# musevlt/muse-psfr

Measured on AMD Instinct MI355X. Metric: PSFs/sec (row x lambda) on 512^2 grid, 35 lambda, higher is better.
Workload: dtype f64 PSD->structure function, per-lambda OTF f32 -> split-fp16 MFMA (fp32 accumulate), f64 fit

## Files before the change

muse_psfr_amd/csrc/kernels.h:

```cpp
#pragma once
#include <hip/hip_runtime.h>
#include <stdint.h>

namespace mpsfr {

constexpr int NS = 40;
constexpr int NSH = NS / 2 + 1;
constexpr int KS = 41;
constexpr int NAO = 80;
constexpr int kNH = NAO / 2 + 1;
constexpr int NFIT = 16;
constexpr int NFIT_ELL = 24;
constexpr int NFIT_PSF = 16;
constexpr int NFIT_GROUP = 48;
constexpr int METRIC_MAX = 16;
constexpr int METRIC_HEAD = 8;
constexpr int KHAT = 33 * 64;
constexpr int MAXLGS = 4;

struct TaskPar {
    double r0m53;
    double inv_l0sq;
    double cn2_0;
    double cn2_1;
// ... 110 lines not shown
size_t mf_dminb_bytes(int N, int ntask);
int mf_block_count(int N);
void launch_mf_tables(hipStream_t s, int N, int nl, const LamPar* d_lp, const void* d_tw64,
                      void* d_E, void* d_G);
void launch_mf_tel(hipStream_t s, int N, const void* d_tel, float* d_tl2, float* d_tlb);
void launch_peak_floor(hipStream_t s, int N, int ntask, int ndir, const void* d_D0t, const float* d_tl2, float c2min,
                       float tier_half, float floor_nominal, float* d_thrf);
void launch_otf_mfma(hipStream_t s, int N, int ntask, int ndir, int nl, const void* d_D0t,
                     const float* d_tl2, const LamPar* d_lp, const void* d_E, const void* d_G,
                     const int* d_vkeep, const float* d_dminb, const float* d_tlb, float thr,
                     void* d_pre, const int* d_order = nullptr, void* d_clk = nullptr, const float* d_thrf = nullptr);
size_t mf2_own_bytes(int N, int ntask, int nl);
size_t mf2_uni_bytes(int N, int ntask, int nl);
size_t mf2_sched_bytes(int N, int ntask, int nl, int permax);
size_t mf2_part_bytes(int N, int ntask, int nl);
void mf2_groups(int nl, int permax, int* per, int* ngr);
void launch_mf_prep(hipStream_t s, int N, int ntask, int nl, int permax, const LamPar* d_lp,
                    const float* d_dminb, const float* d_tlb, float thr, float thr_floor, float thr_mid,
                    float tier_half, const void* d_D0t, const float* d_tl2, void* d_own,
                    void* d_uni, void* d_sched, const float* d_dlin = nullptr);
void launch_otf_mfma2(hipStream_t s, int N, int ntask, int nl, int permax, int ncu, const void* d_D0t,
                      const float* d_tl2, const LamPar* d_lp, const void* d_E, const void* d_G,
                      const void* d_own, const void* d_uni, void* d_sched, void* d_part, void* d_pre,
                      void* d_clk = nullptr, hipEvent_t ev_start = nullptr, hipEvent_t ev_stop = nullptr);
void launch_gtable(hipStream_t s, int N, int nl, const LamPar* d_lp, const void* d_tw64,
                   int* d_samp_p, void* d_samp_a, void* d_G, bool f64);
void launch_moffat_kernels(hipStream_t s, int nker, const double* d_gamma, const double* d_alpha,
                           void* d_out, bool f64);
void launch_otf_rowfft(hipStream_t s, int N, int ntask, int ndir, int nl, const void* d_D0t,
                       const void* d_tel, const LamPar* d_lp, const int* d_samp_p,
                       const void* d_samp_a, const void* d_xtab, void* d_Tq, const void* d_tw64,
                       bool f64, bool fast_exp, const int* d_vkeep);
bool otf_uses_r16(int N, bool f64, int nl, int ndir);
size_t xtab_bytes(int nl);
void launch_xtab(hipStream_t s, int N, int nl, const int* d_samp_p, const void* d_samp_a,
                 const void* d_tw64, void* d_xtab);
void launch_colpass(hipStream_t s, int N, int ntask, int nl, const void* d_Tq, const void* d_G,
                    void* d_pre, bool f64, const int* d_vkeep);
void launch_conv(hipStream_t s, int ntask, int nl, const void* d_pre, const void* d_ktt,
                 const void* d_kmuse, double* d_fin, bool f64, int tdiv = 1);
void launch_khat(hipStream_t s, int nker, const double* d_gamma, const double* d_alpha,
                 void* d_khat, bool f64 = false);
void launch_conv_fft(hipStream_t s, int ntask, int nl, const void* d_pre, const void* d_khat_tt,
                     const void* d_khat_muse, void* d_fin, bool fin_f32, bool f64 = false, int tdiv = 1);
void launch_fit(hipStream_t s, int nstamp, const void* d_stamps, bool stamps_f32, double* d_fit,
                bool f64, int sum_ntask = 0, int sum_nl = 0, double* d_sum = nullptr, int sum_accumulate = 0);
void launch_stamp_sum(hipStream_t s, int ntask, int nl, const void* d_fin, bool fin_f32, double* d_sum,
                      int accumulate);
void launch_fit_ell(hipStream_t s, int nstamp, const double* d_stamps, double* d_fit, bool f64);
void launch_fit_obs(hipStream_t s, int nstamp, const double* d_stamps, const double* d_var, int flags, double* d_fit,
                    bool f64);
void launch_fit_psf(hipStream_t s, int nstamp, const double* d_stamps, const double* d_var, int npsf,
                    const double* d_psf, const int32_t* d_index, const double* d_shift, int flags, double* d_fit,
                    bool f64);
void launch_fit_group(hipStream_t s, int nstamp, int nsrc, const double* d_stamps, const double* d_var, int npsf,
                      const double* d_psf, const int32_t* d_index, const double* d_shift, int flags, double* d_fit,
                      bool f64);
void launch_fit_spec(hipStream_t s, int nstar, int nl, const double* d_cubes, const double* d_var, int npsf,
                     const double* d_psf, const int32_t* d_index, const double* d_shift, const double* d_x, int flags,
                     double* d_fit, bool f64);
void launch_stamp_metrics(hipStream_t s, int nstamp, const double* d_stamps, const double* d_centers, int nrad,
                          const double* radii, int nbox, const double* boxes, int nfrac, const double* fractions,
                          double* d_out);
void launch_cut_stamps(hipStream_t s, int ny, int nx, const double* d_image, const double* d_var, int nstar,
                       const int32_t* d_origin, double* d_stamps, double* d_var_out);
struct StarList {
    int nstar, npsf;
// ... 59 lines not shown
```

muse_psfr_amd/csrc/mf_common.h:

```cpp
#pragma once
#include "device_common.h"

namespace mpsfr {
namespace {

typedef _Float16 h8 __attribute__((ext_vector_type(8)));
typedef _Float16 h4 __attribute__((ext_vector_type(4)));
typedef _Float16 h2 __attribute__((ext_vector_type(2)));
typedef float f4 __attribute__((ext_vector_type(4)));
typedef float f2 __attribute__((ext_vector_type(2)));

constexpr int MTL = 16;
constexpr int KBL = 32;
constexpr int NCT = 3;
constexpr int NJT = 2;
constexpr float kShift = 15.0f;
constexpr int kTabShift = 9;

__host__ __device__ constexpr int mf_nks(int N) { return N / KBL; }
__host__ __device__ constexpr int mf_nmt(int N) { return (N / 2 + 1 + MTL - 1) / MTL; }

[[maybe_unused]] __device__ __forceinline__ void split16(float x, _Float16* hi, _Float16* lo) {
    const _Float16 h = (_Float16)x;
    *hi = h;
    *lo = (_Float16)(x - (float)h);
}

[[maybe_unused]] __device__ __forceinline__ f4 mm16(f4 c, h4 ahi, h4 alo, h4 bhi, h4 blo) {
    c = __builtin_amdgcn_mfma_f32_16x16x16f16(alo, bhi, c, 0, 0, 0);
    c = __builtin_amdgcn_mfma_f32_16x16x16f16(ahi, blo, c, 0, 0, 0);
    return __builtin_amdgcn_mfma_f32_16x16x16f16(ahi, bhi, c, 0, 0, 0);
}

[[maybe_unused]] __device__ __forceinline__ void write_stamp(const f4* P0, const f4* Q0, const f4* R2x,
                                                            const f4* R2y, int lr, int lk,
                                                            float* __restrict__ out) {
    float va[2 * NJT * 4], vb[2 * NJT * 4];
    float part = 0.f;
#pragma unroll
    for (int jt = 0; jt < NJT; ++jt) {
        const int jj = 16 * jt + lr;
        const bool jok = jj < NSH;
        const float mj = (jj >= 1 && jj <= NS / 2 - 1) ? 1.f : 0.f;
#pragma unroll
        for (int r = 0; r < 4; ++r) {
            const float qhi = __shfl_xor(R2y[jt][r], 32, 64);
#pragma unroll
            for (int top = 0; top < 2; ++top) {
                const int row = 4 * lk + r;
                const int ii = top ? 16 + row : row;
                const bool ok = jok && (top ? row < 5 : true);
                const float Pv = top ? R2x[jt][r] : P0[jt][r];
                const float Qv = top ? qhi : Q0[jt][r];
                const float pa = ok ? fmaxf(Pv + Qv, 0.f) : 0.f;
                const float pb = ok ? fmaxf(Pv - Qv, 0.f) : 0.f;
                const float mi = (ii >= 1 && ii <= NS / 2 - 1) ? 1.f : 0.f;
                part += pa * (1.f + mi * mj) + pb * (mi + mj);
                va[(top * NJT + jt) * 4 + r] = pa;
                vb[(top * NJT + jt) * 4 + r] = pb;
            }
        }
    }
    const double tot = wave_sum((double)part);
    const float inv = (float)(1.0 / tot);
#pragma unroll
    for (int top = 0; top < 2; ++top)
#pragma unroll
        for (int jt = 0; jt < NJT; ++jt)
#pragma unroll
            for (int r = 0; r < 4; ++r) {
                const int row = 4 * lk + r, ii = top ? 16 + row : row, jj = 16 * jt + lr;
                if (jj >= NSH || (top && row >= 5)) continue;
                const float pa = va[(top * NJT + jt) * 4 + r] * inv, pb = vb[(top * NJT + jt) * 4 + r] * inv;
                const bool mi = ii >= 1 && ii <= NS / 2 - 1, mj = jj >= 1 && jj <= NS / 2 - 1;
                out[ii * NS + jj] = pa;
                if (mi) out[(NS - ii) * NS + jj] = pb;
                if (mj) out[ii * NS + NS - jj] = pb;
                if (mi && mj) out[(NS - ii) * NS + NS - jj] = pa;
            }
}

[[maybe_unused]] __device__ __forceinline__ bool part_col(int jt, int lr) { return 16 * jt + lr < NSH; }
[[maybe_unused]] __device__ __forceinline__ bool part_r2x(int lk) { return lk < 2; }
[[maybe_unused]] __device__ __forceinline__ bool part_r2y(int lk) { return lk >= 2; }

constexpr int kT2 = 8;

#ifndef MPSFR_MF_BASE_NOP
#define MPSFR_MF_BASE_NOP 4
#endif
#ifndef MF_XSTR
#define MF_STR(x_) #x_
#define MF_XSTR(x_) MF_STR(x_)
#endif

[[maybe_unused]] __device__ __forceinline__ void glds16s(const void* sbase, unsigned voff, unsigned lds_dst) {
    unsigned keep;
    asm volatile(
        "s_nop " MF_XSTR(MPSFR_MF_BASE_NOP) "\n\ts_mov_b32 %0, m0\n\ts_mov_b32 m0, %3\n\ts_nop 0\n\tglobal_load_lds_dwordx4 %1, %2\n\ts_mov_b32 m0, %0"
        : "=&s"(keep)
        : "v"(voff), "s"(sbase), "s"(lds_dst)
        : "memory");
// ... 27 lines not shown
```

muse_psfr_amd/csrc/mpsfr_api.cpp:

```cpp
#include "../../include/mpsfr.h"

#include <hip/hip_runtime.h>

#include <algorithm>
#include <chrono>
#include <cmath>
#include <cstdarg>
#include <cstdio>
#include <cstring>
#include <string>
#include <thread>
#include <vector>

#include "coeff_l0_table.h"
#include "kernels.h"

using namespace mpsfr;

namespace {

thread_local std::string g_err;

constexpr float kMfFloorLog2 = -29.01f;

// ... 17 lines not shown

const char* kKernelNames[K_COUNT] = {
    "ao_tables", "tel_otf", "psd_rowfft", "colfft_dphi", "gtable",
    "moffat_kernels", "otf_rowfft", "colpass", "conv", "fit", "stamp_sum", "vkeep", "otf_mfma", "mf_prep",
    "patch", "dphi_series"};

struct DevBuf {
    void* p = nullptr;
    size_t cap = 0;
};

struct Pending {
    int id;
    hipEvent_t a, b;
};

}

struct mpsfr_ctx {
    int device = 0, N = 0, dimpsf = 0, prec = 0, ncu = 256;
    int reserve_mf = -1, reserve_a = -1;
    bool head_fusion = true;
    bool support_skip = true;
    double pixscale = 0.2;
    bool f64 = false;
    hipStream_t stream = nullptr;
    int chunk_tasks = 0;
    bool fast_exp = true;
    bool profile = false;
    int prof_only = -1;
    int prof_every = 1;
    unsigned prof_count[64] = {};
    bool fft_conv = true;
    int prune_fixed = 0;
    double prune_eps = 1.0e-9;
    double prune_eps_f64 = 1.0e-13;
    bool otf_mfma = true;
    bool mf_floor = true;
    int mf_kernel = 2;
    int mf_permax = 6;
    double mf_mid_log2 = -18.01;
    double mf_floor_log2 = kMfFloorLog2;
    double tier_eps = 4.0e-6;
    bool mf_clock = false;
    int stage_a = 1;
    DevBuf mfclk;
// ... 84 lines not shown
        std::vector<double> sums;
        std::vector<long> tickets;
        double* user_sum = nullptr;
    } multi;
    long ticket_next = 0;
    long d0t_clears = 0;
    double host_seconds = 0.0;
    long host_calls = 0;
    std::vector<double> cache_lbda;
    int cache_lbda_mode = -1;
    const void* cache_G_ptr = nullptr;
    const void* cache_kmuse_ptr = nullptr;
    const void* cache_xtab_ptr = nullptr;
    bool cache_xtab_valid = false;
    const void* cache_etab_ptr = nullptr;
    const void* cache_gtab_ptr = nullptr;
    bool cache_mf_valid = false;
    std::vector<unsigned char> cache_geom;
    const void* cache_ao_ptr = nullptr;
    int last_ndir = 0, last_nl = 0, last_chunk_tasks = 0, last_lane = 0;
    int last_ntab = 2;
    int last_gpp = 1;
    bool last_mf = false, last_pruned = false, last_mf2 = false, last_dlin = false;
    float last_thr_blk = 0.f;
    bool last_floor_per_task = false;
    std::vector<double> last_lpc;
    float last_thr[7] = {0.f, 0.f, 0.f, 0.f, 0.f, 0.f, 0.f};
    double prof_ms[K_COUNT] = {0};
    long prof_n[K_COUNT] = {0};
    std::vector<Pending> pending;
    std::vector<hipEvent_t> pool;
};

namespace {

size_t rsize(const mpsfr_ctx* c) { return c->f64 ? sizeof(double) : sizeof(float); }

int ensure(mpsfr_ctx* c, DevBuf& b, size_t bytes) {
    if (bytes <= b.cap) return MPSFR_OK;
    if (b.p) {
        HIPCHK(hipDeviceSynchronize());
        HIPCHK(hipFree(b.p));
        b.p = nullptr;
        b.cap = 0;
    }
    const size_t want = bytes + bytes / 8;
// ... 495 lines not shown
    } else if (!strcmp(key, "prune_eps")) {
        if (!(value >= 0.0) || value > 1.0e-3) return fail(MPSFR_E_INVALID, "prune_eps must be in [0, 1e-3]");
        c->prune_eps = value;
    } else if (!strcmp(key, "otf_mfma")) {
        c->otf_mfma = value != 0.0;
    } else if (!strcmp(key, "mf_floor")) {
        c->mf_floor = value != 0.0;
    } else if (!strcmp(key, "mf_kernel")) {
        if (value != 1.0 && value != 2.0) return fail(MPSFR_E_INVALID, "mf_kernel must be 1 or 2");
        c->mf_kernel = (int)value;
    } else if (!strcmp(key, "cold_stagger")) {
        c->cold_stagger = (int)value;
    } else if (!strcmp(key, "mf_permax")) {
        if (value != (int)value || value < 1.0 || value > 7.0) return fail(MPSFR_E_INVALID, "mf_permax must be 1..7");
        c->mf_permax = (int)value;
    } else if (!strcmp(key, "persist_reserve") || !strcmp(key, "persist_reserve_mf") || !strcmp(key, "persist_reserve_a")) {
        if (value != (int)value || value < -1.0 || value > 128.0) return fail(MPSFR_E_INVALID, "%s must be -1 (automatic) or 0..128", key);
        if (key[15] == '\0' || key[16] == 'm') c->reserve_mf = (int)value;
        if (key[15] == '\0' || key[16] == 'a') c->reserve_a = (int)value;
    } else if (!strcmp(key, "support_skip")) {
        c->support_skip = value != 0.0;
    } else if (!strcmp(key, "head_fusion")) {
        c->head_fusion = value != 0.0;
    } else if (!strcmp(key, "param_copy")) {
        c->param_copy_kernel = value != 0.0;
    } else if (!strcmp(key, "tier_eps")) {
        if (!(value >= 0.0)) return fail(MPSFR_E_INVALID, "tier_eps must be >= 0 (inf: tiers without a budget)");
        c->tier_eps = value;
    } else if (!strcmp(key, "mf_floor_log2")) {
        c->mf_floor_log2 = value;
    } else if (!strcmp(key, "mf_mid_log2")) {
        c->mf_mid_log2 = value;
    } else if (!strcmp(key, "stage_a")) {
        if (value != 0.0 && value != 1.0 && value != 2.0)
            return fail(MPSFR_E_INVALID, "stage_a must be 0 (full-size transforms), 1 (automatic) or 2 (series + patch)");
        c->stage_a = (int)value;
    } else if (!strcmp(key, "mf_clock")) {
        c->mf_clock = value != 0.0;
        if (c->mf_clock) {
            const int rc = ensure(c, c->mfclk, (size_t)65536 * 8 * 8 * sizeof(unsigned long long));
            if (rc) return rc;
            HIPCHK(hipMemset(c->mfclk.p, 0, c->mfclk.cap));
        }
    } else if (!strcmp(key, "pipeline_calls")) {
        c->pipeline_calls = value != 0.0;
    } else if (!strcmp(key, "fft_conv")) {
// ... 1033 lines not shown
        }
        if (!c->lsum_done) HIPCHK(hipEventCreateWithFlags(&c->lsum_done, hipEventDisableTiming));
        HIPCHK(hipEventRecord(c->lsum_done, s));
        c->lsum_busy = true;
    }
    if (!m.lean) {
        HIPCHK(hipEventRecord(sl.call_done, s));
        if (!c->stream_tail) HIPCHK(hipEventCreateWithFlags(&c->stream_tail, hipEventDisableTiming));
    }
    sl.call_pending = true;
    sl.last_lane = m.lean ? L.index(0) : -1;
    sl.has_event = !m.zero;
    return MPSFR_OK;
}

static void remember_call(mpsfr_ctx* c, const CallPrep& p, bool dlin) {
    c->last_ndir = p.ndir;
    c->last_gpp = p.gpp;
    c->last_nl = p.nl;
    c->last_mf = p.mf;
    c->last_mf2 = p.mf2;
    c->last_pruned = p.th.prune;
    c->last_dlin = dlin;
    c->last_thr_blk = p.th.thr_blk;
    c->last_floor_per_task = p.th.floor_per_task;
    const float thr[7] = {p.th.thr_eps, p.th.thr_floor, p.th.thr_mid, p.th.tier_half, p.th.thr_blk, p.th.thr_sum,
                          p.th.c2min};
    for (int k = 0; k < 7; ++k) c->last_thr[k] = thr[k];
    c->last_lpc.resize(p.nl);
    for (int l = 0; l < p.nl; ++l) c->last_lpc[l] = p.lp[l].c;
}


struct Chunk {
    int t0, tc;
    int j;
    bool accumulate;
    bool shared;
};

static int d0t_begin(mpsfr_ctx* c, mpsfr_ctx::Lane& ln, bool skip_form, int leaves) {
    if (ln.d0t_stale == 2 || (ln.d0t_stale == 1 && skip_form)) {
        HIPCHK(hipMemsetAsync(ln.D0t.p, 0, ln.D0t.cap, ln.stream));
        ln.d0t_stale = 0;
        ++c->d0t_clears;
    }
// ... 22 lines not shown
            }
            launch_patch(ls, N, ntd, ndir, d.tp + t0, (const double*)c->aotab.p, cfit, c->stwk.p,
                         (double*)ln.pP.p, ln.pT.p, (double*)ln.psp.p, c->f64, kh, d.mix(t0));
        }
        ProfScope ps(c, K_DPHI_SERIES, ls);
        launch_dphi_series(ls, N, ntd, ndir, d.tp + t0, ln.pT.p, (const double*)ln.psp.p, c->scoef.p,
                           c->stwk.p, scale2, ln.D0t.p, p.th.prune ? (float*)ln.dlin.p : nullptr, c->f64,
                           msched, persist_grid(c, ln, c->reserve_a, ck.shared),
                           c->support_skip ? (const unsigned*)c->ssup.p : nullptr);
    } else {
        {
            ProfScope ps(c, K_PSD_ROWFFT, ls);
            launch_psd_rowfft(ls, N, ntd, ndir, d.tp + t0, (const double*)c->aotab.p, cfit, ln.C.p,
                              c->tw64.p, (double*)ln.s00.p, c->f64, d.mix(t0));
        }
        ProfScope ps(c, K_COLFFT_DPHI, ls);
        launch_colfft_dphi(ls, N, ntd, ln.C.p, (const double*)ln.s00.p, scale2, ln.D0t.p,
                           c->f64, c->tw64.p, msched);
    }
    return MPSFR_OK;
}

static int stage_b(mpsfr_ctx* c, mpsfr_ctx::Lane& ln, const CallPrep& p, const DevParams& d, const Chunk& ck,
                   bool from_lines, CallLanes& L) {
    hipStream_t ls = ln.stream;
    const int N = p.N, nl = p.nl, ndb = p.ndb, ntd = ck.tc * p.ndir;
    const int tb = ck.tc * p.gpp;
    const Thresholds& th = p.th;
    const bool prune = th.prune;
    if (p.mf2) {
        ProfScope ps(c, K_MF_PREP, ls);
        const bool lines = prune && from_lines;
        if (prune && !lines) launch_dmin(ls, N, ntd, ln.D0t.p, (float*)ln.dmin.p, (float*)ln.dblk.p);
        launch_mf_prep(ls, N, tb, nl, c->mf_permax, d.lp, (prune && !lines) ? (const float*)ln.dblk.p : nullptr,
                       (const float*)c->tlb.p, th.thr_eps, th.thr_floor, th.thr_mid, th.tier_half, ln.D0t.p,
                       (const float*)c->tl2.p, ln.mown.p, ln.muni.p, ln.msched.p,
                       lines ? (const float*)ln.dlin.p : nullptr);
    } else if (prune) {
        ProfScope ps(c, p.mf ? K_MF_PREP : K_VKEEP, ls);
        if (from_lines) launch_dmin16(ls, N, ntd, (const float*)ln.dlin.p, (float*)ln.dmin.p, (float*)ln.dblk.p);
        else launch_dmin(ls, N, ntd, ln.D0t.p, (float*)ln.dmin.p, (float*)ln.dblk.p, c->f64);
        launch_vkeep(ls, N, tb, ndb, nl, d.lp, (const float*)ln.dmin.p, (const float*)ln.dblk.p,
                     (const float*)c->tlmax.p, th.thr_sum, (int*)ln.vkeep.p, c->prune_fixed,
                     p.mf ? (float*)ln.dminb.p : nullptr);
        if (p.mf) launch_task_order(ls, tb, nl, (const int*)ln.vkeep.p, (int*)ln.order.p);
    }
    const int* d_vkeep = prune ? (const int*)ln.vkeep.p : nullptr;
    if (int rc = stagger_here(c, L, 2, ln)) return rc;
    if (p.mf2) {
        ProfScope ps(c, K_OTF_MFMA, ls, false);
        launch_otf_mfma2(ls, N, tb, nl, c->mf_permax, persist_grid(c, ln, c->reserve_mf, ck.shared), ln.D0t.p,
                         (const float*)c->tl2.p, d.lp, c->etab.p, c->gtab.p, ln.mown.p, ln.muni.p, ln.msched.p,
                         ln.mpart.p, ln.pre.p, c->mf_clock ? c->mfclk.p : nullptr, ps.a, ps.b);
    } else if (p.mf) {
        ProfScope ps(c, K_OTF_MFMA, ls);
        if (th.floor_per_task)
            launch_peak_floor(ls, N, tb, ndb, ln.D0t.p, (const float*)c->tl2.p, th.c2min, th.tier_half, th.thr_floor,
                              (float*)ln.thrf.p);
        launch_otf_mfma(ls, N, tb, ndb, nl, ln.D0t.p, (const float*)c->tl2.p, d.lp, c->etab.p,
                        c->gtab.p, d_vkeep, prune ? (const float*)ln.dminb.p : nullptr,
                        (const float*)c->tlb.p, th.thr_blk, ln.pre.p,
                        prune ? (const int*)ln.order.p : nullptr, c->mf_clock ? c->mfclk.p : nullptr,
                        th.floor_per_task ? (const float*)ln.thrf.p : nullptr);
    } else {
        {
            ProfScope ps(c, K_OTF_ROWFFT, ls);
            launch_otf_rowfft(ls, N, tb, ndb, nl, ln.D0t.p, c->tel.p, d.lp,
                              (const int*)c->samp_p.p, c->samp_a.p, c->xtab.p, ln.Tq.p, c->tw64.p,
                              c->f64, c->fast_exp, d_vkeep);
        }
        ProfScope ps(c, K_COLPASS, ls);
        launch_colpass(ls, N, tb, nl, ln.Tq.p, c->G.p, ln.pre.p, c->f64, d_vkeep);
    }
    return MPSFR_OK;
}

static int chunk_tail(mpsfr_ctx* c, mpsfr_ctx::Lane& ln, const CallPrep& p, const DevParams& d, const CallOuts& o,
                      const Chunk& ck, int NL) {
    hipStream_t ls = ln.stream;
    const int nl = p.nl, nsum = p.nsum, t0 = ck.t0, tc = ck.tc;
    const int tb = tc * p.gpp;
    const size_t per_stamp = kStampPix;
    const bool fin_f32 = p.band ? (p.fft_conv && !c->f64)
                                : (p.fft_conv && !c->f64 && !o.d_fin_all && !(o.psf && !o.dev));
    void* d_fin = o.d_fin_all ? (void*)(o.d_fin_all + (size_t)t0 * nsum * per_stamp) : ln.fin.p;
    {
        ProfScope ps(c, K_CONV, ls);
        const char* ktt = d.ktt + (size_t)t0 * p.ksz;
        if (p.fft_conv) launch_conv_fft(ls, tb, nl, ln.pre.p, ktt, c->kmuse.p, d_fin, fin_f32, c->f64, p.gpp);
        else launch_conv(ls, tb, nl, ln.pre.p, ktt, c->kmuse.p, (double*)d_fin, c->f64, p.gpp);
    }
    void* d_res = d_fin;
    bool res_f32 = fin_f32;
    if (p.band) {
        ProfScope ps(c, K_STAMP_SUM, ls);
        double* d_band = (o.dev && o.psf) ? o.psf + (size_t)t0 * nsum * per_stamp : (double*)ln.band.p;
        launch_band_reduce(ls, tb, nl, p.nout, d_fin, fin_f32, d.bw, d_band);
        d_res = d_band;
        res_f32 = false;
    }
    double* lsum = !o.sum ? nullptr : NL > 1 ? (double*)c->lsum.p + (size_t)ck.j * nsum * per_stamp : o.d_sum;
    if (o.fit) {
        ProfScope ps(c, K_FIT, ls);
        launch_fit(ls, tb * p.nout, d_res, res_f32, o.d_fit_all + (size_t)t0 * nsum * NFIT, c->f64,
                   o.sum ? tc : 0, nsum, o.sum ? lsum : nullptr, ck.accumulate ? 1 : 0);
    } else if (o.sum) {
        ProfScope ps(c, K_STAMP_SUM, ls);
        launch_stamp_sum(ls, tc, nsum, d_res, res_f32, lsum, ck.accumulate ? 1 : 0);
    }
    HIPCHK(hipGetLastError());
    if (!o.dev && o.psf) {
        HIPCHK(hipMemcpyAsync(o.psf + (size_t)t0 * nsum * per_stamp, d_res,
                              (size_t)tc * nsum * per_stamp * sizeof(double), hipMemcpyDeviceToHost, ls));
// ... 31 lines not shown
    mpsfr_ctx::Ticket* tk = nullptr;
    if (a.on_device == 2 && (rc = ticket_begin(c, p, o, tk))) return rc;
    const bool pipelined = c->pipeline_calls && o.dev;
    CallLanes L;
    if ((rc = lanes_begin(c, p.ntask, pipeline_chunk_tasks(c, p, !pipelined), pipelined, L))) return rc;
    const Markers marks(c, o.dev, tk != nullptr, L.NL);
    hipStream_t s0 = L.at(c, 0).stream;
    std::vector<unsigned char> ao_key = ao_cache_key(p.g, p.ly, a.mask_rec, a.mask_res);
    bool ao_cached = false, lam_cached = false;
    if ((rc = size_ao_tables(c, p, ao_key, ao_cached))) return rc;
    const Blob blob(p, a.mask_rec && !ao_cached);
    mpsfr_ctx::Slot* sl = nullptr;
    if ((rc = slot_acquire(c, blob.bytes, (size_t)p.ntask * p.ksz, sl, clock.blocked))) return rc;
    blob.fill(sl->host, p, a.mask_rec, a.mask_res);
    const void* outs[3] = {o.dev ? (const void*)o.psf : nullptr, o.dev ? (const void*)o.sum : nullptr,
                           o.dev ? (const void*)o.fit : nullptr};
    if ((rc = queue_call_waits(c, L, *sl, outs))) return rc;
    const std::vector<double> lb_key(a.lbda_nm, a.lbda_nm + a.nl);
    if ((rc = size_wavelength_tables(c, p, lb_key, lam_cached))) return rc;
    if ((rc = send_params(c, *sl, s0, blob.bytes, marks))) return rc;
    const DevParams d = blob.views(*sl, p);
    if ((rc = refresh_tables(c, s0, p, d, ao_cached ? nullptr : &ao_key, lam_cached ? nullptr : &lb_key))) return rc;
    const bool fuse_khat = c->head_fusion && p.series && p.fft_conv;
    launch_tiptilt(c, s0, p, d, *sl, fuse_khat);
    for (int j = 0; j < L.NL; ++j)
        if ((rc = size_lane(c, L.at(c, j), p, L.TC, STAGE_A | STAGE_B | STAGE_TAIL, p.band && !(o.dev && o.psf))))
            return rc;
    if ((rc = size_outputs(c, p, L.NL, o))) return rc;
    if ((rc = share_tables(c, L))) return rc;
    rc = for_each_chunk(c, p.ntask, L, lanes_are_shared(c, L), [&](mpsfr_ctx::Lane& ln, const Chunk& ck) {
        int r;
        if ((r = stage_a(c, ln, p, d, ck, fuse_khat))) return r;
        if ((r = stagger_here(c, L, 1, ln))) return r;
        if ((r = stage_b(c, ln, p, d, ck, p.th.prune && p.series, L))) return r;
        return chunk_tail(c, ln, p, d, o, ck, L.NL);
    });
    if (rc) return rc;
    if ((rc = call_end(c, L, *sl, marks, outs, p.nsum, o.sum ? o.d_sum : nullptr))) return rc;
    remember_call(c, p, p.th.prune && p.series);
    if (tk && (rc = ticket_finish(c, tk))) return rc;
    if (!o.dev) {
        hipStream_t s = c->stream;
        if (o.fit)
            HIPCHK(hipMemcpyAsync(o.fit, o.d_fit_all, (size_t)p.ntask * p.nsum * NFIT * sizeof(double),
                                  hipMemcpyDeviceToHost, s));
        if (o.sum)
            HIPCHK(hipMemcpyAsync(o.sum, o.d_sum, (size_t)p.nsum * kStampPix * sizeof(double), hipMemcpyDeviceToHost, s));
        HIPCHK(hipStreamSynchronize(s));
    }
    clock.finish(c);
    return MPSFR_OK;
}

struct ScopedBuf : DevBuf {
    ~ScopedBuf() { release(*this); }
};

enum : unsigned { TABLES_AO = 1, TABLES_WAVELENGTH = 2 };
static const void* const kNoOuts[3] = {nullptr, nullptr, nullptr};

struct StageCall {
    CallLanes L;
// ... 1040 lines not shown
    if (!strcmp(what, "ao_tables")) {
        n = (size_t)2 * c->last_ndir * (c->last_ntab + 1) * NAO * NAO;
        src = c->aotab.p;
    } else if (!strcmp(what, "tel")) {
        n = (size_t)H1 * N;
        src = c->tel.p;
        is_real_r = true;
    } else if (!strcmp(what, "dphi0")) {
        n = (size_t)c->last_chunk_tasks * c->last_ndir * H1 * N;
        src = c->lane[c->last_lane].D0t.p;
        is_real_r = true;
    } else if (!strcmp(what, "dlin")) {
        if (!c->last_dlin)
            return fail(MPSFR_E_INVALID, "no line minima in the last call (prune_eps = 0, or stage A did not run in "
                                         "its series form)");
        n = (size_t)c->last_chunk_tasks * c->last_ndir * H1 * (N / 32);
        if (n > capacity) return fail(MPSFR_E_INVALID, "capacity %zu < %zu", capacity, n);
        std::vector<float> tmp(n);
        HIPCHK(hipMemcpy(tmp.data(), c->lane[c->last_lane].dlin.p, n * sizeof(float), hipMemcpyDeviceToHost));
        for (size_t i = 0; i < n; ++i) out[i] = (double)tmp[i];
        return (long)n;
    } else if (!strcmp(what, "pre")) {
        n = (size_t)c->last_chunk_tasks * c->last_gpp * c->last_nl * NS * NS;
        src = c->lane[c->last_lane].pre.p;
        is_real_r = true;
    } else if (!strcmp(what, "mf_work")) {
        if (capacity < 3) return fail(MPSFR_E_INVALID, "capacity %zu < 3", capacity);
        if (!c->last_mf) return fail(MPSFR_E_INVALID, "the last call did not use the matrix-core kernel");
        const int tc = c->last_chunk_tasks * c->last_gpp, nl = c->last_nl, npair = (nl + 1) / 2;
        const int nks = N / 32, nmt = (H1 + 15) / 16, nb = nmt * nks;
        const mpsfr_ctx::Lane& ln = c->lane[c->last_lane];
        std::vector<int> vk((size_t)tc * npair);
        std::vector<float> dm((size_t)tc * nb), tb((size_t)nb);
        if (c->last_pruned && !c->last_mf2) {
            HIPCHK(hipMemcpy(vk.data(), ln.vkeep.p, vk.size() * sizeof(int), hipMemcpyDeviceToHost));
            HIPCHK(hipMemcpy(dm.data(), ln.dminb.p, dm.size() * sizeof(float), hipMemcpyDeviceToHost));
            HIPCHK(hipMemcpy(tb.data(), c->tlb.p, tb.size() * sizeof(float), hipMemcpyDeviceToHost));
        }
        double steps = 0.0, tiles = 0.0, steps_full = 0.0, steps_mid = 0.0, steps_union = -1.0, steps_support = -1.0;
        if (c->last_mf2) {
            std::vector<unsigned long long> own((size_t)tc * nl * nmt * 2);
            HIPCHK(hipMemcpy(own.data(), ln.mown.p, own.size() * sizeof(unsigned long long), hipMemcpyDeviceToHost));
            for (size_t i = 0; i < own.size(); i += 2) {
                const int nf = __builtin_popcountll(own[i]), nm = __builtin_popcountll(own[i + 1]);
                steps_full += nf;
                steps_mid += nm;
                tiles += (nf + nm) > 0;
// ... 236 lines not shown
```

muse_psfr_amd/csrc/otf_mfma2.hip:

```cpp
#include <hip/hip_ext.h>
#include "mf_common.h"

namespace mpsfr {

namespace {

typedef unsigned long long u64;

constexpr int kTW = 4;
constexpr int kStage2 = kT2 * 4096;
constexpr int kSlab = 6 * 1024;

struct MaskArgs {
    int N, nl, per, ngr;
    const LamPar* lp;
    const float* dminb;
    const float* dlin;
    const float* tlb;
    float thr, thr_mid;
    float thr_floor, tier_half;
    const float* D0t;
    const float* tl2;
    u64* own;
    u64* uni;
// ... 616 lines not shown
                    const float* d_dminb, const float* d_tlb, float thr, float thr_floor, float thr_mid,
                    float tier_half, const void* d_D0t, const float* d_tl2, void* d_own,
                    void* d_uni, void* d_sched, const float* d_dlin) {
    MaskArgs a;
    a.dlin = d_dlin;
    a.thr_floor = thr_floor; a.tier_half = tier_half;
    a.D0t = (const float*)d_D0t; a.tl2 = d_tl2;
    a.N = N; a.nl = nl;
    mf2_groups(nl, permax, &a.per, &a.ngr);
    a.lp = d_lp; a.dminb = d_dminb; a.tlb = d_tlb;
    a.thr = thr; a.thr_mid = thr_mid;
    a.own = (u64*)d_own; a.uni = (u64*)d_uni;
    a.ksum = a.uni + (size_t)ntask * nl * mf_nmt(N);
    a.kuni = a.ksum + (size_t)ntask * nl * mf2_nsw(N);
    const SchedPtrs p = sched_ptrs(d_sched, ntask, nl);
    a.gsw = p.gsw; a.sched = p.sched; a.items = p.items;
    a.cap = (int)mf2_cap(N, ntask, a.ngr);
    hipLaunchKernelGGL(k_mf_prep, dim3(a.ngr, ntask), dim3(64 * a.per), 0, s, a);
}

void launch_otf_mfma2(hipStream_t s, int N, int ntask, int nl, int permax, int ncu, const void* d_D0t,
                      const float* d_tl2, const LamPar* d_lp, const void* d_E, const void* d_G,
                      const void* d_own, const void* d_uni, void* d_sched, void* d_part, void* d_pre,
                      void* d_clk, hipEvent_t ev_start, hipEvent_t ev_stop) {
    Mf2Args a;
    a.N = N; a.ntask = ntask; a.nl = nl;
    mf2_groups(nl, permax, &a.per, &a.ngr);
    a.D0t = (const float*)d_D0t; a.tl2 = d_tl2; a.lp = d_lp;
    a.E = (const h8*)d_E; a.G = (const h4*)d_G;
    a.own = (const u64*)d_own; a.uni = (const u64*)d_uni;
    a.ksum = a.uni + (size_t)ntask * nl * mf_nmt(N);
    a.kuni = a.ksum + (size_t)ntask * nl * mf2_nsw(N);
    const SchedPtrs p = sched_ptrs(d_sched, ntask, nl);
    a.sched = p.sched; a.items = p.items;
    a.cap = (int)mf2_cap(N, ntask, a.ngr);
    a.part = (f4*)d_part;
    a.clk = (unsigned long long*)d_clk;
    int lg = 0;
    while ((1 << lg) < N) ++lg;
    a.tq_scale = 1.0f / ((float)(1 << lg) * (float)(1 << kTabShift));
    a.pre = (float*)d_pre;
    const int maxitems = ntask * a.ngr * (int)mf2_nsw(N);
    const int nwg = ncu < maxitems ? ncu : maxitems;
    const size_t sm = 2 * (size_t)kStage2 + 2 * (size_t)a.per * kSlab + 64;
    if (permax > 6) {
        allow_smem(k_otf_mfma2<4>, 2 * (size_t)kStage2 + 2 * (size_t)7 * kSlab + 64);
        if (ev_start != nullptr)
            hipExtLaunchKernelGGL(k_otf_mfma2<4>, dim3(nwg), dim3(128 * a.per), (unsigned)sm, s, ev_start, ev_stop, 0, a);
        else
            hipLaunchKernelGGL(k_otf_mfma2<4>, dim3(nwg), dim3(128 * a.per), sm, s, a);
    } else {
        allow_smem(k_otf_mfma2<3>, 2 * (size_t)kStage2 + 2 * (size_t)6 * kSlab + 64);
        if (ev_start != nullptr)
            hipExtLaunchKernelGGL(k_otf_mfma2<3>, dim3(nwg), dim3(128 * a.per), (unsigned)sm, s, ev_start, ev_stop, 0, a);
        else
            hipLaunchKernelGGL(k_otf_mfma2<3>, dim3(nwg), dim3(128 * a.per), sm, s, a);
    }
    hipLaunchKernelGGL(k_mf_finish, dim3(nl, ntask), dim3(64), 0, s, N, nl, a.per, a.ngr, (const int*)p.gsw,
                       (const f4*)a.part, a.pre);
}

}
```

muse_psfr_amd/csrc/stamps.hip:

```cpp
#include "device_common.h"
#include "conv_frames.h"
#include "fit_common.h"
#include <type_traits>

namespace mpsfr {

namespace {

template <typename R>
__global__ void __launch_bounds__(256)
k_moffat_kernels(const double* __restrict__ gam, const double* __restrict__ alp,
                 R* __restrict__ out) {
    __shared__ double part[4];
    __shared__ double tot;
    const int k = blockIdx.x;
    const double g2 = gam[k] * gam[k], al = alp[k];
    double vals[(KS * KS + 255) / 256];
    double s = 0.0;
#pragma unroll
    for (int m = 0; m < (KS * KS + 255) / 256; ++m) {
        const int e = threadIdx.x + m * 256;
        double v = 0.0;
        if (e < KS * KS) {
            const int dy = e / KS - KS / 2, dx = e % KS - KS / 2;
            const double x1 = 1.0 + (double)(dx * dx + dy * dy) / g2;
// ... 76 lines not shown
            const R* __restrict__ krow = kg + a * KS;
#pragma unroll
            for (int b = 0; b < KS; ++b) {
                const R kv = krow[b];
#pragma unroll
                for (int o = 0; o < SW; ++o) part[o] += kv * sv[o - b + 2 * HK];
            }
#pragma unroll
            for (int o = 0; o < SW; ++o) acc[o] += (double)part[o];
        }
        __syncthreads();
        if (pass == 0 && active) {
#pragma unroll
            for (int o = 0; o < SW; ++o) img[(i + HK) * PW + j0 + HK + o] = (R)acc[o];
        }
    }
    if (active) {
        double* out = fin + ((size_t)task * nl + l) * NS * NS + i * NS + j0;
#pragma unroll
        for (int o = 0; o < SW; ++o) out[o] = acc[o];
    }
}

template <typename R, typename TF>
#ifndef MPSFR_CONV_WAVES
#define MPSFR_CONV_WAVES 4
#endif
__global__ void __launch_bounds__(256) __attribute__((amdgpu_waves_per_eu(sizeof(R) == 4 ? MPSFR_CONV_WAVES : 2)))
k_conv_fft(int nl, int tdiv, const R* __restrict__ pre, const cx<R>* __restrict__ khat_tt,
           const cx<R>* __restrict__ khat_muse, TF* __restrict__ fin) {
    extern __shared__ __align__(16) unsigned char conv_smem[];
    cx<R> (*F)[CFP] = reinterpret_cast<cx<R> (*)[CFP]>(conv_smem);
    cx<R> (*bufs)[CFB] = reinterpret_cast<cx<R> (*)[CFB]>(conv_smem + sizeof(cx<R>) * CF * CFP);
    const int l = blockIdx.x, task = blockIdx.y;
    const int slot = threadIdx.x >> 3, t = threadIdx.x & 7;
    Tw64<R> tw;
    tw.init(t);
    const R* src = pre + ((size_t)task * nl + l) * NS * NS;
    cx<R>* buf = bufs[slot];
    cx<R> x[8];
#pragma unroll
    for (int e = 0; e < 8; ++e) {
        const int c = t + 8 * e;
        const bool in = c < NS && slot < NS / 2;
        x[e] = {in ? src[2 * slot * NS + c] : (R)0, in ? src[(2 * slot + 1) * NS + c] : (R)0};
    }
    for (int pass = 0; pass < 2; ++pass) {
        const cx<R>* __restrict__ kh = pass == 0 ? khat_tt + (size_t)(task / tdiv) * (CFH + 1) * CF
                                                     : khat_muse + (size_t)l * (CFH + 1) * CF;
        cx<R> khv[8], khn[8];
#pragma unroll
        for (int e = 0; e < 8; ++e) {
            khv[e] = kh[slot * CF + t + 8 * e];
            khn[e] = slot == 0 ? kh[CFH * CF + t + 8 * e] : cx<R>{(R)0, (R)0};
        }
        __syncthreads();
        if (slot < NS / 2) cf_rows_forward(x, F, buf, tw, slot, t);
        __syncthreads();
        {
            static_assert(fft_last_nbt<CF>() == 1 && fft_last_radix<CF>() == 8, "v[e] is element t + 8 e");
            cx<R> y[8], xin[8], v[8];
#pragma unroll
            for (int e = 0; e < 8; ++e) {
                const int r = t + 8 * e;
                xin[e] = r < NS ? F[r][slot] : cx<R>{(R)0, (R)0};
            }
            fft_forward_regs_lastreg<R, CF, true>(xin, buf, buf, tw.w, t, v);
            if (slot == 0) {
// ... 651 lines not shown
                           (const double*)d_kmuse, d_fin);
    } else {
        const size_t sm = (size_t)(PH * PW) * sizeof(float);
        hipLaunchKernelGGL(k_conv<float>, grid, dim3(256), sm, s, nl, tdiv, (const float*)d_pre,
                           (const float*)d_ktt,
                           (const float*)d_kmuse, d_fin);
    }
}

void launch_khat(hipStream_t s, int nker, const double* d_gamma, const double* d_alpha,
                 void* d_khat, bool f64) {
    if (nker <= 0) return;
    if (f64) {
        allow_smem(k_khat<double>, conv_smem_bytes<double>(true));
        hipLaunchKernelGGL(k_khat<double>, dim3(nker), dim3(256), conv_smem_bytes<double>(true), s, d_gamma,
                           d_alpha, (cx<double>*)d_khat);
    } else {
        hipLaunchKernelGGL(k_khat<float>, dim3(nker), dim3(256), conv_smem_bytes<float>(true), s, d_gamma,
                           d_alpha, (cx<float>*)d_khat);
    }
}

void launch_conv_fft(hipStream_t s, int ntask, int nl, const void* d_pre, const void* d_khat_tt,
                     const void* d_khat_muse, void* d_fin, bool fin_f32, bool f64, int tdiv) {
    const dim3 grid(nl, ntask);
    if (f64) {
        allow_smem((k_conv_fft<double, double>), conv_smem_bytes<double>(false));
        hipLaunchKernelGGL((k_conv_fft<double, double>), grid, dim3(256), conv_smem_bytes<double>(false), s, nl, tdiv,
                           (const double*)d_pre, (const cx<double>*)d_khat_tt, (const cx<double>*)d_khat_muse,
                           (double*)d_fin);
    } else if (fin_f32) {
        hipLaunchKernelGGL((k_conv_fft<float, float>), grid, dim3(256), conv_smem_bytes<float>(false), s, nl, tdiv,
                           (const float*)d_pre, (const cx<float>*)d_khat_tt, (const cx<float>*)d_khat_muse,
                           (float*)d_fin);
    } else {
        hipLaunchKernelGGL((k_conv_fft<float, double>), grid, dim3(256), conv_smem_bytes<float>(false), s, nl, tdiv,
                           (const float*)d_pre, (const cx<float>*)d_khat_tt, (const cx<float>*)d_khat_muse,
                           (double*)d_fin);
    }
}

void launch_fit(hipStream_t s, int nstamp, const void* d_stamps, bool stamps_f32, double* d_fit,
                bool f64, int sum_ntask, int sum_nl, double* d_sum, int sum_accumulate) {
    if (nstamp <= 0) return;
    SumArgs sa = {0, sum_ntask, sum_nl, sum_accumulate, d_sum};
    if (d_sum != nullptr && sum_ntask > 0) {
        const size_t per = (size_t)sum_nl * NS * NS;
        sa.nwg = (int)((per + 64 * MPSFR_FIT_WG - 1) / (64 * MPSFR_FIT_WG));
    }
    const dim3 grid(sa.nwg + (nstamp + MPSFR_FIT_WG - 1) / MPSFR_FIT_WG), blk(64 * MPSFR_FIT_WG);
#ifndef MPSFR_FIT_F64_LM
#define MPSFR_FIT_F64_LM 0
#endif
    if (f64 && MPSFR_FIT_F64_LM)
        hipLaunchKernelGGL((k_fit<double, double>), grid, blk, 0, s, nstamp,
                           (const double*)d_stamps, d_fit, 0.0, sa);
    else if (stamps_f32)
        hipLaunchKernelGGL((k_fit<float, float>), grid, blk, 0, s, nstamp, (const float*)d_stamps,
                           d_fit, (double)MPSFR_POLISH_TOL, sa);
    else
        hipLaunchKernelGGL((k_fit<float, double>), grid, blk, 0, s, nstamp,
// ... 18 lines not shown
```

Before: 20.53 million.

## Fuse MFMA partial-tile reduction into the FFT convolution kernel

The separate k_mf_finish kernel, which summed per-sweep partial tiles into the pre stamps, is removed from the default path. When mf2 and the FFT convolution are both active in f32 mode and outputs stay on the host, the convolution kernel reads the partial tiles itself, reduces them in shared memory and writes the stamp there before its FFT. This saves one kernel launch and the global round trip through pre. A debug readout of 'pre' now runs the finish lazily, and there is extra shared-memory and register pressure in the convolution kernel.

```diff
diff --git a/muse_psfr_amd/csrc/kernels.h b/muse_psfr_amd/csrc/kernels.h
--- a/muse_psfr_amd/csrc/kernels.h
+++ b/muse_psfr_amd/csrc/kernels.h
@@ -156,7 +156,16 @@
 void launch_otf_mfma2(hipStream_t s, int N, int ntask, int nl, int permax, int ncu, const void* d_D0t,
                       const float* d_tl2, const LamPar* d_lp, const void* d_E, const void* d_G,
                       const void* d_own, const void* d_uni, void* d_sched, void* d_part, void* d_pre,
-                      void* d_clk = nullptr, hipEvent_t ev_start = nullptr, hipEvent_t ev_stop = nullptr);
+                      void* d_clk = nullptr, hipEvent_t ev_start = nullptr, hipEvent_t ev_stop = nullptr,
+                      bool finish = true);
+void launch_mf_finish(hipStream_t s, int N, int ntask, int nl, int permax, const void* d_sched, const void* d_part,
+                      void* d_pre);
+struct MfPartial {
+    const void* part;
+    const int* gsw;
+    int per, ngr, nsw;
+};
+MfPartial mf2_partial(int N, int ntask, int nl, int permax, const void* d_sched, const void* d_part);
 void launch_gtable(hipStream_t s, int N, int nl, const LamPar* d_lp, const void* d_tw64,
                    int* d_samp_p, void* d_samp_a, void* d_G, bool f64);
 void launch_moffat_kernels(hipStream_t s, int nker, const double* d_gamma, const double* d_alpha,
@@ -176,7 +185,8 @@
 void launch_khat(hipStream_t s, int nker, const double* d_gamma, const double* d_alpha,
                  void* d_khat, bool f64 = false);
 void launch_conv_fft(hipStream_t s, int ntask, int nl, const void* d_pre, const void* d_khat_tt,
-                     const void* d_khat_muse, void* d_fin, bool fin_f32, bool f64 = false, int tdiv = 1);
+                     const void* d_khat_muse, void* d_fin, bool fin_f32, bool f64 = false, int tdiv = 1,
+                     const MfPartial* tiles = nullptr);
 void launch_fit(hipStream_t s, int nstamp, const void* d_stamps, bool stamps_f32, double* d_fit,
                 bool f64, int sum_ntask = 0, int sum_nl = 0, double* d_sum = nullptr, int sum_accumulate = 0);
 void launch_stamp_sum(hipStream_t s, int ntask, int nl, const void* d_fin, bool fin_f32, double* d_sum,
diff --git a/muse_psfr_amd/csrc/mf_common.h b/muse_psfr_amd/csrc/mf_common.h
--- a/muse_psfr_amd/csrc/mf_common.h
+++ b/muse_psfr_amd/csrc/mf_common.h
@@ -34,7 +34,7 @@
 
 [[maybe_unused]] __device__ __forceinline__ void write_stamp(const f4* P0, const f4* Q0, const f4* R2x,
                                                             const f4* R2y, int lr, int lk,
-                                                            float* __restrict__ out) {
+                                                            float* __restrict__ out, int share = 0, int nshare = 1) {
     float va[2 * NJT * 4], vb[2 * NJT * 4];
     float part = 0.f;
 #pragma unroll
@@ -66,7 +66,8 @@
 #pragma unroll
     for (int top = 0; top < 2; ++top)
 #pragma unroll
-        for (int jt = 0; jt < NJT; ++jt)
+        for (int jt = 0; jt < NJT; ++jt) {
+            if (nshare > 1 && (top * NJT + jt) % nshare != share) continue;
 #pragma unroll
             for (int r = 0; r < 4; ++r) {
                 const int row = 4 * lk + r, ii = top ? 16 + row : row, jj = 16 * jt + lr;
@@ -78,6 +79,7 @@
                 if (mj) out[ii * NS + NS - jj] = pb;
                 if (mi && mj) out[(NS - ii) * NS + NS - jj] = pa;
             }
+        }
 }
 
 [[maybe_unused]] __device__ __forceinline__ bool part_col(int jt, int lr) { return 16 * jt + lr < NSH; }
diff --git a/muse_psfr_amd/csrc/mpsfr_api.cpp b/muse_psfr_amd/csrc/mpsfr_api.cpp
--- a/muse_psfr_amd/csrc/mpsfr_api.cpp
+++ b/muse_psfr_amd/csrc/mpsfr_api.cpp
@@ -63,6 +63,7 @@
     int reserve_mf = -1, reserve_a = -1;
     bool head_fusion = true;
     bool support_skip = true;
+    int finish_in_conv = -1;
     double pixscale = 0.2;
     bool f64 = false;
     hipStream_t stream = nullptr;
@@ -193,6 +194,7 @@
     int last_ntab = 2;
     int last_gpp = 1;
     bool last_mf = false, last_pruned = false, last_mf2 = false, last_dlin = false;
+    bool last_unfinished = false;
     float last_thr_blk = 0.f;
     bool last_floor_per_task = false;
     std::vector<double> last_lpc;
@@ -734,6 +736,10 @@
         c->support_skip = value != 0.0;
     } else if (!strcmp(key, "head_fusion")) {
         c->head_fusion = value != 0.0;
+    } else if (!strcmp(key, "finish_in_conv")) {
+        if (value != -1.0 && value != 0.0 && value != 1.0)
+            return fail(MPSFR_E_INVALID, "finish_in_conv must be -1 (automatic), 0 or 1");
+        c->finish_in_conv = (int)value;
     } else if (!strcmp(key, "param_copy")) {
         c->param_copy_kernel = value != 0.0;
     } else if (!strcmp(key, "tier_eps")) {
@@ -1813,6 +1819,7 @@
     c->last_mf2 = p.mf2;
     c->last_pruned = p.th.prune;
     c->last_dlin = dlin;
+    c->last_unfinished = false;
     c->last_thr_blk = p.th.thr_blk;
     c->last_floor_per_task = p.th.floor_per_task;
     const float thr[7] = {p.th.thr_eps, p.th.thr_floor, p.th.thr_mid, p.th.tier_half, p.th.thr_blk, p.th.thr_sum,
@@ -1881,7 +1888,7 @@
 }
 
 static int stage_b(mpsfr_ctx* c, mpsfr_ctx::Lane& ln, const CallPrep& p, const DevParams& d, const Chunk& ck,
-                   bool from_lines, CallLanes& L) {
+                   bool from_lines, CallLanes& L, bool finish = true) {
     hipStream_t ls = ln.stream;
     const int N = p.N, nl = p.nl, ndb = p.ndb, ntd = ck.tc * p.ndir;
     const int tb = ck.tc * p.gpp;
@@ -1910,7 +1917,7 @@
         ProfScope ps(c, K_OTF_MFMA, ls, false);
         launch_otf_mfma2(ls, N, tb, nl, c->mf_permax, persist_grid(c, ln, c->reserve_mf, ck.shared), ln.D0t.p,
                          (const float*)c->tl2.p, d.lp, c->etab.p, c->gtab.p, ln.mown.p, ln.muni.p, ln.msched.p,
-                         ln.mpart.p, ln.pre.p, c->mf_clock ? c->mfclk.p : nullptr, ps.a, ps.b);
+                         ln.mpart.p, ln.pre.p, c->mf_clock ? c->mfclk.p : nullptr, ps.a, ps.b, finish);
     } else if (p.mf) {
         ProfScope ps(c, K_OTF_MFMA, ls);
         if (th.floor_per_task)
@@ -1935,7 +1942,7 @@
 }
 
 static int chunk_tail(mpsfr_ctx* c, mpsfr_ctx::Lane& ln, const CallPrep& p, const DevParams& d, const CallOuts& o,
-                      const Chunk& ck, int NL) {
+                      const Chunk& ck, int NL, bool from_tiles = false) {
     hipStream_t ls = ln.stream;
     const int nl = p.nl, nsum = p.nsum, t0 = ck.t0, tc = ck.tc;
     const int tb = tc * p.gpp;
@@ -1946,8 +1953,14 @@
     {
         ProfScope ps(c, K_CONV, ls);
         const char* ktt = d.ktt + (size_t)t0 * p.ksz;
-        if (p.fft_conv) launch_conv_fft(ls, tb, nl, ln.pre.p, ktt, c->kmuse.p, d_fin, fin_f32, c->f64, p.gpp);
-        else launch_conv(ls, tb, nl, ln.pre.p, ktt, c->kmuse.p, (double*)d_fin, c->f64, p.gpp);
+        if (p.fft_conv) {
+            MfPartial tiles = {};
+            if (from_tiles) tiles = mf2_partial(p.N, tb, nl, c->mf_permax, ln.msched.p, ln.mpart.p);
+            launch_conv_fft(ls, tb, nl, ln.pre.p, ktt, c->kmuse.p, d_fin, fin_f32, c->f64, p.gpp,
+                            from_tiles ? &tiles : nullptr);
+        } else {
+            launch_conv(ls, tb, nl, ln.pre.p, ktt, c->kmuse.p, (double*)d_fin, c->f64, p.gpp);
+        }
     }
     void* d_res = d_fin;
     bool res_f32 = fin_f32;
@@ -2025,6 +2038,8 @@
     const DevParams d = blob.views(*sl, p);
     if ((rc = refresh_tables(c, s0, p, d, ao_cached ? nullptr : &ao_key, lam_cached ? nullptr : &lb_key))) return rc;
     const bool fuse_khat = c->head_fusion && p.series && p.fft_conv;
+    const bool tiles_to_conv = p.mf2 && p.fft_conv && !c->f64 &&
+                               (c->finish_in_conv > 0 || (c->finish_in_conv < 0 && !o.dev));
     launch_tiptilt(c, s0, p, d, *sl, fuse_khat);
     for (int j = 0; j < L.NL; ++j)
         if ((rc = size_lane(c, L.at(c, j), p, L.TC, STAGE_A | STAGE_B | STAGE_TAIL, p.band && !(o.dev && o.psf))))
@@ -2035,12 +2050,13 @@
         int r;
         if ((r = stage_a(c, ln, p, d, ck, fuse_khat))) return r;
         if ((r = stagger_here(c, L, 1, ln))) return r;
-        if ((r = stage_b(c, ln, p, d, ck, p.th.prune && p.series, L))) return r;
-        return chunk_tail(c, ln, p, d, o, ck, L.NL);
+        if ((r = stage_b(c, ln, p, d, ck, p.th.prune && p.series, L, !tiles_to_conv))) return r;
+        return chunk_tail(c, ln, p, d, o, ck, L.NL, tiles_to_conv);
     });
     if (rc) return rc;
     if ((rc = call_end(c, L, *sl, marks, outs, p.nsum, o.sum ? o.d_sum : nullptr))) return rc;
     remember_call(c, p, p.th.prune && p.series);
+    c->last_unfinished = tiles_to_conv;
     if (tk && (rc = ticket_finish(c, tk))) return rc;
     if (!o.dev) {
         hipStream_t s = c->stream;
@@ -3127,7 +3143,15 @@
         return (long)n;
     } else if (!strcmp(what, "pre")) {
         n = (size_t)c->last_chunk_tasks * c->last_gpp * c->last_nl * NS * NS;
-        src = c->lane[c->last_lane].pre.p;
+        mpsfr_ctx::Lane& ln = c->lane[c->last_lane];
+        if (c->last_unfinished) {
+            launch_mf_finish(ln.stream, N, c->last_chunk_tasks * c->last_gpp, c->last_nl, c->mf_permax, ln.msched.p,
+                             ln.mpart.p, ln.pre.p);
+            HIPCHK(hipGetLastError());
+            HIPCHK(hipStreamSynchronize(ln.stream));
+            c->last_unfinished = false;
+        }
+        src = ln.pre.p;
         is_real_r = true;
     } else if (!strcmp(what, "mf_work")) {
         if (capacity < 3) return fail(MPSFR_E_INVALID, "capacity %zu < 3", capacity);
diff --git a/muse_psfr_amd/csrc/otf_mfma2.hip b/muse_psfr_amd/csrc/otf_mfma2.hip
--- a/muse_psfr_amd/csrc/otf_mfma2.hip
+++ b/muse_psfr_amd/csrc/otf_mfma2.hip
@@ -662,7 +662,7 @@
 void launch_otf_mfma2(hipStream_t s, int N, int ntask, int nl, int permax, int ncu, const void* d_D0t,
                       const float* d_tl2, const LamPar* d_lp, const void* d_E, const void* d_G,
                       const void* d_own, const void* d_uni, void* d_sched, void* d_part, void* d_pre,
-                      void* d_clk, hipEvent_t ev_start, hipEvent_t ev_stop) {
+                      void* d_clk, hipEvent_t ev_start, hipEvent_t ev_stop, bool finish) {
     Mf2Args a;
     a.N = N; a.ntask = ntask; a.nl = nl;
     mf2_groups(nl, permax, &a.per, &a.ngr);
@@ -696,8 +696,23 @@
         else
             hipLaunchKernelGGL(k_otf_mfma2<3>, dim3(nwg), dim3(128 * a.per), sm, s, a);
     }
-    hipLaunchKernelGGL(k_mf_finish, dim3(nl, ntask), dim3(64), 0, s, N, nl, a.per, a.ngr, (const int*)p.gsw,
-                       (const f4*)a.part, a.pre);
-}
-
-}
+    if (finish) launch_mf_finish(s, N, ntask, nl, permax, d_sched, d_part, d_pre);
+}
+
+MfPartial mf2_partial(int N, int ntask, int nl, int permax, const void* d_sched, const void* d_part) {
+    MfPartial t;
+    t.part = d_part;
+    t.gsw = sched_ptrs(const_cast<void*>(d_sched), ntask, nl).gsw;
+    mf2_groups(nl, permax, &t.per, &t.ngr);
+    t.nsw = (int)mf2_nsw(N);
+    return t;
+}
+
+void launch_mf_finish(hipStream_t s, int N, int ntask, int nl, int permax, const void* d_sched, const void* d_part,
+                      void* d_pre) {
+    const MfPartial t = mf2_partial(N, ntask, nl, permax, d_sched, d_part);
+    hipLaunchKernelGGL(k_mf_finish, dim3(nl, ntask), dim3(64), 0, s, N, nl, t.per, t.ngr, t.gsw, (const f4*)t.part,
+                       (float*)d_pre);
+}
+
+}
diff --git a/muse_psfr_amd/csrc/stamps.hip b/muse_psfr_amd/csrc/stamps.hip
--- a/muse_psfr_amd/csrc/stamps.hip
+++ b/muse_psfr_amd/csrc/stamps.hip
@@ -1,6 +1,7 @@
 #include "device_common.h"
 #include "conv_frames.h"
 #include "fit_common.h"
+#include "mf_common.h"
 #include <type_traits>
 
 namespace mpsfr {
@@ -123,28 +124,107 @@
     }
 }
 
-template <typename R, typename TF>
+struct ConvPart {
+    const f4* part;
+    const int* gsw;
+    int per, ngr, nsw;
+};
+constexpr int kFinTileBytes = 4 * NJT * 64 * (int)sizeof(f4);
+constexpr int kFinBatch = 6;
+static_assert(NJT == 2, "a thread takes the tiles w and 4 + w: both of column tile w & 1");
+static_assert(kFinTileBytes + NS * NS * (int)sizeof(float) <= (int)sizeof(cx<float>) * CF * CFP, "the scratch lives in F");
+
+__device__ __forceinline__ void conv_finish_intake(const ConvPart& cp, int m, int task, int nl, int l,
+                                                   unsigned char* smem) {
+    f4* tiles = reinterpret_cast<f4*>(smem);
+    float* stamp = reinterpret_cast<float*>(smem + kFinTileBytes);
+    const int lane = threadIdx.x & 63, w = threadIdx.x >> 6;
+    const bool col = part_col(w & 1, lane & 15);
+    const bool top = col && (w < 2 ? part_r2x(lane >> 4) : part_r2y(lane >> 4));
+    const f4* pt = cp.part + ((size_t)task * nl + l) * cp.nsw * (4 * NJT * 64);
+    const unsigned e0 = threadIdx.x, e1 = threadIdx.x + 4 * 64;
+    const f4 z = {0.f, 0.f, 0.f, 0.f};
+    int mm = m & ((1 << cp.nsw) - 1);
+    const int n = __builtin_popcount(mm);
+    f4 a[kFinBatch], b[kFinBatch];
+#pragma unroll
+    for (int k = 0; k < kFinBatch; ++k) {
+        const f4* ps = pt + (size_t)(mm != 0 ? __builtin_ctz(mm) : 0) * (4 * NJT * 64);
+        mm &= mm - 1;
+        a[k] = (col && k < n) ? ps[e0] : z;
+        b[k] = (top && k < n) ? ps[e1] : z;
+    }
+    f4 s0 = a[0], s1 = b[0];
+#pragma unroll
+    for (int k = 1; k < kFinBatch; ++k) {
+        const f4 t0 = s0 + a[k], t1 = s1 + b[k];
+        s0 = k < n ? t0 : s0;
+        s1 = k < n ? t1 : s1;
+    }
+#pragma clang loop unroll(disable)
+    while (mm != 0) {
+        const f4* ps = pt + (size_t)__builtin_ctz(mm) * (4 * NJT * 64);
+        mm &= mm - 1;
+        s0 = s0 + (col ? ps[e0] : z);
+        s1 = s1 + (top ? ps[e1] : z);
+    }
+    tiles[threadIdx.x] = s0;
+    tiles[4 * 64 + threadIdx.x] = s1;
+    __syncthreads();
+    {
+        f4 P0[NJT], Q0[NJT], R2x[NJT], R2y[NJT];
+#pragma unroll
+        for (int jt = 0; jt < NJT; ++jt) {
+            P0[jt] = tiles[(0 * NJT + jt) * 64 + lane];
+            Q0[jt] = tiles[(1 * NJT + jt) * 64 + lane];
+            R2x[jt] = tiles[(2 * NJT + jt) * 64 + lane];
+            R2y[jt] = tiles[(3 * NJT + jt) * 64 + lane];
+        }
+        write_stamp(P0, Q0, R2x, R2y, lane & 15, lane >> 4, stamp, w, 4);
+    }
+    __syncthreads();
+}
+
+template <typename R, typename TF, bool FIN = false>
 #ifndef MPSFR_CONV_WAVES
 #define MPSFR_CONV_WAVES 4
 #endif
 __global__ void __launch_bounds__(256) __attribute__((amdgpu_waves_per_eu(sizeof(R) == 4 ? MPSFR_CONV_WAVES : 2)))
 k_conv_fft(int nl, int tdiv, const R* __restrict__ pre, const cx<R>* __restrict__ khat_tt,
-           const cx<R>* __restrict__ khat_muse, TF* __restrict__ fin) {
+           const cx<R>* __restrict__ khat_muse, TF* __restrict__ fin, ConvPart cp) {
+    static_assert(!FIN || sizeof(R) == 4, "partial tiles are a mixed-mode matter");
     extern __shared__ __align__(16) unsigned char conv_smem[];
     cx<R> (*F)[CFP] = reinterpret_cast<cx<R> (*)[CFP]>(conv_smem);
     cx<R> (*bufs)[CFB] = reinterpret_cast<cx<R> (*)[CFB]>(conv_smem + sizeof(cx<R>) * CF * CFP);
     const int l = blockIdx.x, task = blockIdx.y;
     const int slot = threadIdx.x >> 3, t = threadIdx.x & 7;
     Tw64<R> tw;
-    tw.init(t);
+    if constexpr (!FIN) tw.init(t);
+    cx<R>* buf = bufs[slot];
     const R* src = pre + ((size_t)task * nl + l) * NS * NS;
-    cx<R>* buf = bufs[slot];
+    bool from_tiles = false;
+    if constexpr (FIN) {
+        const int m = cp.gsw[task * cp.ngr + l / cp.per];
+        from_tiles = __builtin_popcount(m) > 1;
+        if (from_tiles) conv_finish_intake(cp, m, task, nl, l, conv_smem);
+        tw.init(t);
+    }
     cx<R> x[8];
-#pragma unroll
-    for (int e = 0; e < 8; ++e) {
-        const int c = t + 8 * e;
-        const bool in = c < NS && slot < NS / 2;
-        x[e] = {in ? src[2 * slot * NS + c] : (R)0, in ? src[(2 * slot + 1) * NS + c] : (R)0};
+    if (from_tiles) {
+        const R* st = reinterpret_cast<const R*>(conv_smem + kFinTileBytes);
+#pragma unroll
+        for (int e = 0; e < 8; ++e) {
+            const int c = t + 8 * e;
+            const bool in = c < NS && slot < NS / 2;
+            x[e] = {in ? st[2 * slot * NS + c] : (R)0, in ? st[(2 * slot + 1) * NS + c] : (R)0};
+        }
+    } else {
+#pragma unroll
+        for (int e = 0; e < 8; ++e) {
+            const int c = t + 8 * e;
+            const bool in = c < NS && slot < NS / 2;
+            x[e] = {in ? src[2 * slot * NS + c] : (R)0, in ? src[(2 * slot + 1) * NS + c] : (R)0};
+        }
     }
     for (int pass = 0; pass < 2; ++pass) {
         const cx<R>* __restrict__ kh = pass == 0 ? khat_tt + (size_t)(task / tdiv) * (CFH + 1) * CF
@@ -842,21 +922,32 @@
 }
 
 void launch_conv_fft(hipStream_t s, int ntask, int nl, const void* d_pre, const void* d_khat_tt,
-                     const void* d_khat_muse, void* d_fin, bool fin_f32, bool f64, int tdiv) {
+                     const void* d_khat_muse, void* d_fin, bool fin_f32, bool f64, int tdiv, const MfPartial* tiles) {
     const dim3 grid(nl, ntask);
+    ConvPart cp = {nullptr, nullptr, 1, 1, 0};
+    if (tiles != nullptr && !f64) cp = {(const f4*)tiles->part, tiles->gsw, tiles->per, tiles->ngr, tiles->nsw};
     if (f64) {
         allow_smem((k_conv_fft<double, double>), conv_smem_bytes<double>(false));
         hipLaunchKernelGGL((k_conv_fft<double, double>), grid, dim3(256), conv_smem_bytes<double>(false), s, nl, tdiv,
                            (const double*)d_pre, (const cx<double>*)d_khat_tt, (const cx<double>*)d_khat_muse,
-                           (double*)d_fin);
+                           (double*)d_fin, cp);
+    } else if (cp.part != nullptr) {
+        if (fin_f32)
+            hipLaunchKernelGGL((k_conv_fft<float, float, true>), grid, dim3(256), conv_smem_bytes<float>(false), s, nl,
+                               tdiv, (const float*)d_pre, (const cx<float>*)d_khat_tt, (const cx<float>*)d_khat_muse,
+                               (float*)d_fin, cp);
+        else
+            hipLaunchKernelGGL((k_conv_fft<float, double, true>), grid, dim3(256), conv_smem_bytes<float>(false), s, nl,
+                               tdiv, (const float*)d_pre, (const cx<float>*)d_khat_tt, (const cx<float>*)d_khat_muse,
+                               (double*)d_fin, cp);
     } else if (fin_f32) {
         hipLaunchKernelGGL((k_conv_fft<float, float>), grid, dim3(256), conv_smem_bytes<float>(false), s, nl, tdiv,
                            (const float*)d_pre, (const cx<float>*)d_khat_tt, (const cx<float>*)d_khat_muse,
-                           (float*)d_fin);
+                           (float*)d_fin, cp);
     } else {
         hipLaunchKernelGGL((k_conv_fft<float, double>), grid, dim3(256), conv_smem_bytes<float>(false), s, nl, tdiv,
                            (const float*)d_pre, (const cx<float>*)d_khat_tt, (const cx<float>*)d_khat_muse,
-                           (double*)d_fin);
+                           (double*)d_fin, cp);
     }
 }
 
```

Result: no change. 20.48 million (-0.2%).
